# paninski-lab/eks

Hardware: AMD Instinct MI355X
Metric: frames*keypoints smoothed/s + achieved HBM GB/s fraction, singlecam 100k x 256 (higher is better)
Workload: dtype f32

## Files before the change

### eks_amd/csrc/eks_diag.hip

```cpp
#include <hip/hip_runtime.h>

#include <cstdlib>

#include "eks_diag_lane.hpp"
#include "eks_internal.hpp"

namespace eks {

struct LaneMap {
  int N, T, nc;
  int nt_log2;
  int ntile;
  int reverse;
};

__device__ __forceinline__ bool lane_coords(const LaneMap& L, int& n, int& j) {
  const int wave = blockIdx.x * (blockDim.x >> 6) + (threadIdx.x >> 6);
  const int lane = threadIdx.x & 63;
  const int tile = wave % L.ntile;
  const int cg = wave / L.ntile;
  const int nt = 1 << L.nt_log2;
  n = tile * nt + (lane & (nt - 1));
  j = cg * (64 >> L.nt_log2) + (lane >> L.nt_log2);
  return n < L.N && j < L.nc;
// ... 125 lines not shown
  }
  float eta = 0.f, J = 0.f;
  const int npass = (S.nblk + 63) / 64;
  for (int pass = npass - 1; pass >= 0; --pass) {
    const int q0 = pass * 64;
    const Elem<float> own = agg(q0 + lane);
    Elem<float> r = own;
#pragma unroll
    for (int off = 1; off < 64; off <<= 1) {
      const Elem<float> dn = shfl_down_elem(r, off);
      if (lane + off < 64) r = elem_combine(r, dn);
    }
    Elem<float> after = shfl_down_elem(r, 1);
    if (lane == 63) after = elem_identity<float>();
    float eq = eta, Jq = J;
    elem_back(after, eq, Jq);
    if (q0 + lane < S.nblk) {
      const size_t o = (size_t)(q0 + lane) * N + n;
      S.bEta[o] = eq;
      S.bJ[o] = Jq;
    }
    const Elem<float> all{__shfl(r.A, 0), __shfl(r.b, 0), __shfl(r.C, 0), __shfl(r.eta, 0), __shfl(r.J, 0)};
    elem_back(all, eta, J);
  }
}

__global__ __launch_bounds__(kScanCH* kScanCB) void diag_scan_local_kernel(int N, int nc, DiagWs W,
                                                                          ScanWs S) {
  __shared__ ScanLds L;
  const int cl = threadIdx.x % kScanCH, i = threadIdx.x / kScanCH;
  const int n = blockIdx.x * kScanCH + cl, j = blockIdx.y * kScanCB + i;
  const bool live = n < N && j < nc;
  L.put(i, cl, live ? load_elem(W, (size_t)j * N + n) : elem_identity<float>());
  __syncthreads();
  const int w = threadIdx.x >> 6, lane = threadIdx.x & 63;
  const Elem<float> own = L.get(lane, w);
  Elem<float> f = own, r = own;
#pragma unroll
  for (int off = 1; off < kScanCB; off <<= 1) {
    const Elem<float> up = shfl_up_elem(f, off), dn = shfl_down_elem(r, off);
    if (lane >= off) f = elem_combine(up, f);
    if (lane + off < kScanCB) r = elem_combine(r, dn);
  }
  Elem<float> excl = shfl_up_elem(f, 1), after = shfl_down_elem(r, 1);
  if (lane == 0) excl = elem_identity<float>();
  if (lane == kScanCB - 1) after = elem_identity<float>();
  const int nw = blockIdx.x * kScanCH + w;
  float m = 0.f, P = 0.f, eta = 0.f, J = 0.f;
  if (nw < N) {
    const size_t ob = (size_t)blockIdx.y * N + nw;
    m = S.bm[ob];
    P = S.bP[ob];
    eta = S.bEta[ob];
    J = S.bJ[ob];
  }
  elem_apply(excl, m, P);
  elem_back(after, eta, J);
  __syncthreads();
  L.A[lane][w] = m;
  L.b[lane][w] = P;
  L.C[lane][w] = eta;
  L.eta[lane][w] = J;
  __syncthreads();
  if (!live) return;
  const size_t o = (size_t)j * N + n;
  W.pm[o] = L.A[i][cl];
  W.pP[o] = L.b[i][cl];
  W.sEta[o] = L.C[i][cl];
  W.sJ[o] = L.eta[i][cl];
}

constexpr int kFW = 4;
static_assert(kFW == 4, "the fused kernels' LDS exchange, the group scan's slot sizes and the measured "
                        "thresholds in diag_smooth() assume four chunks per block");

struct BlockMap {
  int N, T, nc;
  int ntile;
  int ngrp;
  int reverse;
  int tile0;
};

struct BufferRows {
  __amdgpu_buffer_rsrc_t ry, rv;
  unsigned voff, row_bytes;
  __device__ __forceinline__ float load_y(int i) const {
    return __builtin_bit_cast(float, __builtin_amdgcn_raw_buffer_load_b32(ry, voff, (unsigned)i * row_bytes, 0));
  }
  __device__ __forceinline__ float load_var(int i) const {
    return __builtin_bit_cast(float, __builtin_amdgcn_raw_buffer_load_b32(rv, voff, (unsigned)i * row_bytes, 0));
  }
};

__device__ __forceinline__ __amdgpu_buffer_rsrc_t rows_rsrc(const float* base) {
  return __builtin_amdgcn_make_buffer_rsrc(const_cast<float*>(base), 0, 0x7FFFFFFF, 0x00020000);
}

constexpr int kAuxNt = 2;

template <int VS_ROW>
struct BufferStore {
  __amdgpu_buffer_rsrc_t rm, rV;
  unsigned voff, row_bytes;
  int d;
  __device__ __forceinline__ void operator()(int i, float m, float P) const {
    constexpr unsigned W = VS_ROW == 0 ? 1 : VS_ROW;
    const unsigned so = (unsigned)i * row_bytes;
    __builtin_amdgcn_raw_buffer_store_b32(__builtin_bit_cast(unsigned, m), rm, voff, so, kAuxNt);
    if constexpr (VS_ROW <= 1) {
      __builtin_amdgcn_raw_buffer_store_b32(__builtin_bit_cast(unsigned, P), rV, voff, so, kAuxNt);
    } else if constexpr (VS_ROW == 2) {
      typedef unsigned u2 __attribute__((ext_vector_type(2)));
      const u2 v = {__builtin_bit_cast(unsigned, d == 0 ? P : 0.0f), __builtin_bit_cast(unsigned, d == 1 ? P : 0.0f)};
      __builtin_amdgcn_raw_buffer_store_b64(v, rV, voff * 2, so * 2, kAuxNt);
    } else {
#pragma unroll
      for (unsigned e = 0; e < W; ++e)
        __builtin_amdgcn_raw_buffer_store_b32(__builtin_bit_cast(unsigned, (int)e == d ? P : 0.0f), rV,
                                              voff * W + 4 * e, so * W, kAuxNt);
    }
  }
};

template <int B, bool UNIT, bool RC>
__global__ __launch_bounds__(64 * kFW) void diag_summarize_blk_kernel(BlockMap L, DiagModel M, DiagWs W,
                                                                     ScanWs S,
                                                                     const float* __restrict__ y,
                                                                     const float* __restrict__ var) {
  __shared__ float sh[5][kFW][64];
  __shared__ int arrived;
  const int w = __builtin_amdgcn_readfirstlane(threadIdx.x >> 6), lane = threadIdx.x & 63;
  if (threadIdx.x == 0) arrived = 0;
  __syncthreads();
  const int tile = L.tile0 + blockIdx.x % L.ntile;
  int grp = blockIdx.x / L.ntile;
  if (L.reverse) grp = L.ngrp - 1 - grp;
  const int n = tile * 64 + lane, j = grp * kFW + w;
  Elem<float> e = elem_identity<float>();
  if (n < L.N && j < L.nc) {
    const ChainParams<float> p = load_chain_params(M, n);
    const int t0 = j * B, len = min(B, L.T - t0);
    const size_t first = (size_t)t0 * L.N + (size_t)tile * 64;
    const BufferRows rows{rows_rsrc(y + first), rows_rsrc(var + first), (unsigned)lane * 4, (unsigned)L.N * 4};
    float yy[B], rr[B];
    if (len == B) {
      load_rows<B, true>(rows, B, yy, rr);
      e = summarize_loaded<B, UNIT, true>(yy, rr, B, p);
    } else {
      load_rows<B, false>(rows, len, yy, rr);
      e = summarize_loaded<B, UNIT, false>(yy, rr, len, p);
    }
    if constexpr (!RC) {
      const size_t o = (size_t)j * L.N + n;
      W.eA[o] = e.A;
      W.eb[o] = e.b;
      W.eC[o] = e.C;
      W.eEta[o] = e.eta;
      W.eJ[o] = e.J;
    }
  }
  sh[0][w][lane] = e.A;
  sh[1][w][lane] = e.b;
  sh[2][w][lane] = e.C;
  sh[3][w][lane] = e.eta;
  sh[4][w][lane] = e.J;
  __builtin_amdgcn_fence(__ATOMIC_RELEASE, "workgroup");
  int ticket = 0;
  if (lane == 0) ticket = atomicAdd(&arrived, 1);
  ticket = __builtin_amdgcn_readfirstlane(ticket);
  if (ticket != kFW - 1 || n >= L.N) return;
  __builtin_amdgcn_fence(__ATOMIC_ACQUIRE, "workgroup");
  Elem<float> a{sh[0][0][lane], sh[1][0][lane], sh[2][0][lane], sh[3][0][lane], sh[4][0][lane]};
#pragma unroll
  for (int q = 1; q < kFW; ++q)
    a = elem_combine(a, Elem<float>{sh[0][q][lane], sh[1][q][lane], sh[2][q][lane], sh[3][q][lane],
                                    sh[4][q][lane]});
  const size_t o = (size_t)grp * L.N + n;
  S.gA[o] = a.A;
  S.gb[o] = a.b;
  S.gC[o] = a.C;
  S.gEta[o] = a.eta;
  S.gJ[o] = a.J;
}

template <int B, bool UNIT, int VS_ROW, bool RC>
__global__ __launch_bounds__(64 * kFW) void diag_replay_blk_kernel(BlockMap L, DiagModel M, DiagWs W,
                                                                  ScanWs S,
                                                                  const float* __restrict__ y,
                                                                  const float* __restrict__ var,
                                                                  float* __restrict__ ms,
                                                                  float* __restrict__ Vs) {
  const int w = __builtin_amdgcn_readfirstlane(threadIdx.x >> 6), lane = threadIdx.x & 63;
  const int tile = L.tile0 + blockIdx.x % L.ntile;
  int grp = blockIdx.x / L.ntile;
  if (L.reverse) grp = L.ngrp - 1 - grp;
  const int n = tile * 64 + lane, j = grp * kFW + w;
  const int j0 = grp * kFW, j1 = min(j0 + kFW, L.nc);
  constexpr int VW = VS_ROW == 0 ? 1 : VS_ROW;
  if constexpr (!RC) {
    if (n >= L.N || j >= L.nc) return;
    const ChainParams<float> p = load_chain_params(M, n);
    const int t0 = j * B;
    const int len = min(B, L.T - t0);
    const bool full = len == B;
    const size_t first = (size_t)t0 * L.N + (size_t)tile * 64;
    const BufferRows rows{rows_rsrc(y + first), rows_rsrc(var + first), (unsigned)lane * 4, (unsigned)L.N * 4};
    float v0[B], v1[B];
    if (full) load_rows<B, true>(rows, B, v0, v1);
    else load_rows<B, false>(rows, len, v0, v1);
    Elem<float> ef[kFW - 1];
#pragma unroll
    for (int q = 0; q < kFW - 1; ++q)
      if (j0 + q < j) ef[q] = load_elem(W, (size_t)(j0 + q) * L.N + n);
    const size_t ob = (size_t)grp * L.N + n;
    float m = S.bm[ob], P = S.bP[ob], eta = S.bEta[ob], J = S.bJ[ob];
#pragma unroll
    for (int q = 0; q < kFW - 1; ++q)
      if (j0 + q < j) elem_apply(ef[q], m, P);
    Elem<float> eb[kFW - 1];
#pragma unroll
    for (int q = 0; q < kFW - 1; ++q)
      if (j + 1 + q < j1) eb[q] = load_elem(W, (size_t)(j + 1 + q) * L.N + n);
    if (full) filter_loaded<B, UNIT, true>(v0, v1, B, p, m, P);
    else filter_loaded<B, UNIT, false>(v0, v1, len, p, m, P);
#pragma unroll
    for (int q = kFW - 2; q >= 0; --q)
      if (j + 1 + q < j1) elem_back(eb[q], eta, J);
    fuse_info(m, P, eta, J);
    const BufferStore<VS_ROW> st{rows_rsrc(ms + first), rows_rsrc(Vs + first * VW), (unsigned)lane * 4,
                                 (unsigned)L.N * 4, n % M.D};
    if (full) smooth_rows<B, UNIT, true>(v0, v1, B, p, m, P, st);
    else smooth_rows<B, UNIT, false>(v0, v1, len, p, m, P, st);
  } else {
    __shared__ float sh[5][kFW][64];
    const bool live = n < L.N && j < L.nc;
    ChainParams<float> p{1.f, 1.f, 0.f};
    const int t0 = j < L.nc ? j * B : 0;
    const int len = j < L.nc ? min(B, L.T - t0) : 0;
    const bool full = len == B;
    const size_t first = (size_t)t0 * L.N + (size_t)tile * 64;
    const BufferRows rows{rows_rsrc(y + first), rows_rsrc(var + first), (unsigned)lane * 4, (unsigned)L.N * 4};
    float v0[B], v1[B];
    Elem<float> own = elem_identity<float>();
    if (live) {
      p = load_chain_params(M, n);
      if (full) {
        load_rows<B, true>(rows, B, v0, v1);
        own = summarize_loaded<B, UNIT, true>(v0, v1, B, p);
      } else {
        load_rows<B, false>(rows, len, v0, v1);
        own = summarize_loaded<B, UNIT, false>(v0, v1, len, p);
      }
    }
    sh[0][w][lane] = own.A; sh[1][w][lane] = own.b; sh[2][w][lane] = own.C; sh[3][w][lane] = own.eta;
    sh[4][w][lane] = own.J;
    __syncthreads();
    if (!live) return;
    auto lds_elem = [&](int q) {
      return Elem<float>{sh[0][q][lane], sh[1][q][lane], sh[2][q][lane], sh[3][q][lane], sh[4][q][lane]};
    };
    const size_t ob = (size_t)grp * L.N + n;
    float m = S.bm[ob], P = S.bP[ob], eta = S.bEta[ob], J = S.bJ[ob];
#pragma unroll
    for (int q = 0; q < kFW - 1; ++q)
      if (q < w) elem_apply(lds_elem(q), m, P);
    Elem<float> eb[kFW - 1];
#pragma unroll
    for (int q = 0; q < kFW - 1; ++q)
      if (j + 1 + q < j1) eb[q] = lds_elem(w + 1 + q);
    if (full) filter_loaded<B, UNIT, true>(v0, v1, B, p, m, P);
    else filter_loaded<B, UNIT, false>(v0, v1, len, p, m, P);
#pragma unroll
    for (int q = kFW - 2; q >= 0; --q)
      if (j + 1 + q < j1) elem_back(eb[q], eta, J);
    fuse_info(m, P, eta, J);
    const BufferStore<VS_ROW> st{rows_rsrc(ms + first), rows_rsrc(Vs + first * VW), (unsigned)lane * 4,
                                 (unsigned)L.N * 4, n % M.D};
    if (full) smooth_rows<B, UNIT, true>(v0, v1, B, p, m, P, st);
    else smooth_rows<B, UNIT, false>(v0, v1, len, p, m, P, st);
  }
}

template <int PER, int CH>
__global__ __launch_bounds__(64 * CH) void diag_scan_groups_kernel(int N, int n0, int n1, DiagModel M, ScanWs S) {
  constexpr int NW = CH;
  __shared__ float tot[2][5][NW][CH];
  const int c = threadIdx.x % CH, slot = threadIdx.x / CH, w = threadIdx.x >> 6, lane = threadIdx.x & 63;
  const int lb = xcd_contiguous_block(blockIdx.x, gridDim.x);
  const int n = n0 + lb * CH + c;
  const int per = (S.nblk + 63) / 64;
  const int q0 = min(slot * per, S.nblk), q1 = min(q0 + per, S.nblk);
  const bool live = n < n1;
  auto agg = [&](int q) {
    const size_t o = (size_t)q * N + n;
    return Elem<float>{S.gA[o], S.gb[o], S.gC[o], S.gEta[o], S.gJ[o]};
  };
  Elem<float> own = elem_identity<float>();
  Elem<float> e[PER];
  if (live) {
    for (int b0 = q0; b0 < q1; b0 += PER) {
#pragma unroll
      for (int i = 0; i < PER; ++i)
        if (b0 + i < q1) e[i] = agg(b0 + i);
#pragma unroll
      for (int i = 0; i < PER; ++i)
        if (b0 + i < q1) own = elem_combine(own, e[i]);
    }
  }
  Elem<float> f = own, r = own;
#pragma unroll
  for (int off = CH; off < 64; off <<= 1) {
    const Elem<float> up = shfl_up_elem(f, off), dn = shfl_down_elem(r, off);
    if (lane >= off) f = elem_combine(up, f);
    if (lane + off < 64) r = elem_combine(r, dn);
  }
  if (lane >= 64 - CH) {
    tot[0][0][w][c] = f.A; tot[0][1][w][c] = f.b; tot[0][2][w][c] = f.C; tot[0][3][w][c] = f.eta; tot[0][4][w][c] = f.J;
  }
  if (lane < CH) {
    tot[1][0][w][c] = r.A; tot[1][1][w][c] = r.b; tot[1][2][w][c] = r.C; tot[1][3][w][c] = r.eta; tot[1][4][w][c] = r.J;
  }
  __syncthreads();
  if (!live) return;
  Elem<float> pre = elem_identity<float>(), post = elem_identity<float>();
  for (int v = 0; v < w; ++v)
    pre = elem_combine(pre, Elem<float>{tot[0][0][v][c], tot[0][1][v][c], tot[0][2][v][c], tot[0][3][v][c], tot[0][4][v][c]});
  for (int v = NW - 1; v > w; --v)
    post = elem_combine(Elem<float>{tot[1][0][v][c], tot[1][1][v][c], tot[1][2][v][c], tot[1][3][v][c], tot[1][4][v][c]}, post);
  Elem<float> fe = shfl_up_elem(f, CH), re = shfl_down_elem(r, CH);
  if (lane < CH) fe = elem_identity<float>();
  if (lane >= 64 - CH) re = elem_identity<float>();
  pre = elem_combine(pre, fe);
  post = elem_combine(re, post);
  float m, P;
  load_chain_prior(M, n, m, P);
  elem_apply(pre, m, P);
  float eta = 0.f, J = 0.f;
  elem_back(post, eta, J);
  const bool held = q1 - q0 <= PER;
  for (int b0 = q0; b0 < q1; b0 += PER) {
    if (!held) {
#pragma unroll
      for (int i = 0; i < PER; ++i)
        if (b0 + i < q1) e[i] = agg(b0 + i);
    }
#pragma unroll
    for (int i = 0; i < PER; ++i)
      if (b0 + i < q1) {
        const size_t o = (size_t)(b0 + i) * N + n;
        S.bm[o] = m;
        S.bP[o] = P;
        elem_apply(e[i], m, P);
      }
  }
  for (int b1 = q1; b1 > q0; b1 -= PER) {
    const int lo = max(q0, b1 - PER);
    if (!held) {
#pragma unroll
      for (int i = 0; i < PER; ++i)
        if (lo + i < b1) e[i] = agg(lo + i);
    }
#pragma unroll
    for (int i = PER - 1; i >= 0; --i)
      if (lo + i < b1) {
        const size_t o = (size_t)(lo + i) * N + n;
        S.bEta[o] = eta;
        S.bJ[o] = J;
        elem_back(e[i], eta, J);
      }
  }
}

#ifndef EKS_DIAG_CHUNK
#define EKS_DIAG_CHUNK 32
#endif
constexpr int kChunk = EKS_DIAG_CHUNK;

static inline size_t plane_bytes(int nc, int N) { return align_up((size_t)nc * N * sizeof(float), 256); }

size_t diag_smooth_workspace_bytes(int T, int N) {
  const int nc = (T + kChunk - 1) / kChunk;
  const int nblk = (nc + kFW - 1) / kFW;
  return 9 * plane_bytes(nc, N) + 9 * plane_bytes(nblk, N);
}

static LaneMap make_lane_map(int T, int N, int B) {
  LaneMap L;
  L.N = N;
  L.T = T;
  L.nc = (T + B - 1) / B;
  int nt_log2 = 0;
  while ((1 << nt_log2) < N && nt_log2 < 6) ++nt_log2;
  L.nt_log2 = nt_log2;
  L.ntile = (N + (1 << nt_log2) - 1) >> nt_log2;
  L.reverse = 0;
  return L;
}

template <bool UNIT>
static void launch_replay(int vs_row, dim3 grid, hipStream_t st, const LaneMap& L, const DiagModel& M,
                          const DiagWs& W, const float* y, const float* var, float* ms, float* Vs) {
#define EKS_REPLAY(R)                                                                             \
  case R:                                                                                         \
    hipLaunchKernelGGL((diag_replay_kernel<kChunk, UNIT, R>), grid, dim3(256), 0, st, L, M, W, y, \
                       var, ms, Vs);                                                              \
    break;
  switch (vs_row) {
    EKS_REPLAY(0)
    EKS_REPLAY(1)
    EKS_REPLAY(2)
    EKS_REPLAY(3)
    EKS_REPLAY(4)
    EKS_REPLAY(5)
    EKS_REPLAY(6)
    EKS_REPLAY(7)
    EKS_REPLAY(8)
  }
#undef EKS_REPLAY
}

int diag_smooth(const eks_dims_t& d, const float* y, const float* var, const DiagModel& M,
                float* ms, float* Vs, void* ws, size_t ws_bytes, hipStream_t st) {
  const int T = d.n_frames, D = d.state_dim, N = d.n_keypoints * D;
  const bool vs_diag = d.flags & EKS_FLAG_VS_DIAG;
  if (!vs_diag && D > 8) return EKS_ERR_UNSUPPORTED;
  if (ws_bytes < diag_smooth_workspace_bytes(T, N)) return EKS_ERR_WORKSPACE;
  const LaneMap Lf = make_lane_map(T, N, kChunk);
  const LaneMap& L = Lf;
  const size_t pb = plane_bytes(L.nc, N);
  char* base = static_cast<char*>(ws);
  DiagWs W;
  float** planes[9] = {&W.eA, &W.eb, &W.eC, &W.eEta, &W.eJ, &W.pm, &W.pP, &W.sEta, &W.sJ};
  for (int i = 0; i < 9; ++i) *planes[i] = reinterpret_cast<float*>(base + i * pb);
  const int ngrp_f = (L.nc + kFW - 1) / kFW;
  const bool in_range = (size_t)kChunk * N * (vs_diag ? 1 : D) * sizeof(float) < ((size_t)1 << 31);
  const bool fused = L.nt_log2 == 6 && in_range &&
                     (knob_set(KNOB_SMOOTH_UNFUSED) ? knob_int(KNOB_SMOOTH_UNFUSED, 0) == 0 : ngrp_f <= 1024);
  ScanWs S;
  S.nblk = fused ? (L.nc + kFW - 1) / kFW : (L.nc + kScanCB - 1) / kScanCB;
  const size_t sb = plane_bytes(S.nblk, N);
  float** splanes[9] = {&S.gA, &S.gb, &S.gC, &S.gEta, &S.gJ, &S.bm, &S.bP, &S.bEta, &S.bJ};
  for (int i = 0; i < 9; ++i) *splanes[i] = reinterpret_cast<float*>(base + 9 * pb + i * sb);
  const int vs_row = vs_diag ? 0 : D;
  const bool unit = d.flags & EKS_FLAG_UNIT_AC;
  const int k1_reverse = knob_int(KNOB_SUMMARIZE_REVERSE, 0) == 1 ? 1 : 0;
  const int k3_reverse = knob_set(KNOB_REPLAY_FORWARD) ? (knob_int(KNOB_REPLAY_FORWARD, 0) == 1 ? 0 : 1) : !k1_reverse;
  if (fused) {
    const bool rc_all = knob_set(KNOB_REPLAY_RECOMPUTE) ? knob_int(KNOB_REPLAY_RECOMPUTE, 0) == 1
                                                        : 5 * pb >= ((size_t)16 << 20);
    const int tp = L.ntile;
    for (int tile0 = 0; tile0 < L.ntile; tile0 += tp) {
    const int ntl = min(tp, L.ntile - tile0);
    const int n0 = tile0 * 64, Np = min(N - n0, ntl * 64);
    BlockMap Bm{N, T, L.nc, ntl, S.nblk, k1_reverse, tile0};
    const dim3 bgrid((unsigned)((long)Bm.ntile * Bm.ngrp)), bblock(64 * kFW);
    const bool rc = rc_all;
#define EKS_K1_BLK(UN)                                                                                  \
  do {                                                                                                  \
    if (rc)                                                                                             \
      hipLaunchKernelGGL((diag_summarize_blk_kernel<kChunk, UN, true>), bgrid, bblock, 0, st, Bm, M, W, \
                         S, y, var);                                                                    \
    else                                                                                                \
      hipLaunchKernelGGL((diag_summarize_blk_kernel<kChunk, UN, false>), bgrid, bblock, 0, st, Bm, M,   \
                         W, S, y, var);                                                                 \
  } while (0)
#define EKS_K3_BLK(UN, R)                                                                               \
  do {                                                                                                  \
    if (rc)                                                                                             \
      hipLaunchKernelGGL((diag_replay_blk_kernel<kChunk, UN, R, true>), bgrid, bblock, 0, st, Bm, M, W, \
                         S, y, var, ms, Vs);                                                            \
    else                                                                                                \
      hipLaunchKernelGGL((diag_replay_blk_kernel<kChunk, UN, R, false>), bgrid, bblock, 0, st, Bm, M,   \
                         W, S, y, var, ms, Vs);                                                         \
  } while (0)
    {
      ProfScope ps("diag_summarize", st);
      if (unit)
        EKS_K1_BLK(true);
      else
        EKS_K1_BLK(false);
    }
    {
      ProfScope ps("diag_scan", st);
      const bool ch4 = knob_set(KNOB_SCAN_CH) ? knob_int(KNOB_SCAN_CH, 4) == 4 : Np < 2048;
      const bool per8 = (S.nblk + 63) / 64 <= 8;
      const int Ne = n0 + Np;
      if (ch4) {
        if (per8)
          hipLaunchKernelGGL((diag_scan_groups_kernel<8, 4>), dim3((Np + 3) / 4), dim3(256), 0, st, N, n0, Ne, M, S);
        else
          hipLaunchKernelGGL((diag_scan_groups_kernel<16, 4>), dim3((Np + 3) / 4), dim3(256), 0, st, N, n0, Ne, M, S);
      } else {
        if (per8)
          hipLaunchKernelGGL((diag_scan_groups_kernel<8, 16>), dim3((Np + 15) / 16), dim3(1024), 0, st, N, n0, Ne, M, S);
        else
          hipLaunchKernelGGL((diag_scan_groups_kernel<16, 16>), dim3((Np + 15) / 16), dim3(1024), 0, st, N, n0, Ne, M, S);
      }
    }
    ProfScope ps("diag_replay", st);
    Bm.reverse = k3_reverse;
#define EKS_REPLAY_BLK(R)                                                                              \
  case R:                                                                                              \
    if (unit)                                                                                          \
      EKS_K3_BLK(true, R);                                                                             \
    else                                                                                               \
      EKS_K3_BLK(false, R);                                                                            \
    break;
    switch (vs_row) {
      EKS_REPLAY_BLK(0)
      EKS_REPLAY_BLK(1)
      EKS_REPLAY_BLK(2)
      EKS_REPLAY_BLK(3)
      EKS_REPLAY_BLK(4)
      EKS_REPLAY_BLK(5)
      EKS_REPLAY_BLK(6)
      EKS_REPLAY_BLK(7)
      EKS_REPLAY_BLK(8)
    }
    }
#undef EKS_REPLAY_BLK
#undef EKS_K3_BLK
#undef EKS_K1_BLK
    return hip_status(hipGetLastError());
  }

  const int cpw = 64 >> L.nt_log2;
  const long waves = (long)L.ntile * ((L.nc + cpw - 1) / cpw);
  const dim3 grid((unsigned)((waves + 3) / 4));
  {
    ProfScope ps("diag_summarize", st);
    LaneMap L = Lf;
    L.reverse = k1_reverse;
    if (unit)
      hipLaunchKernelGGL((diag_summarize_kernel<kChunk, true>), grid, dim3(256), 0, st, L, M, W, y, var);
    else
      hipLaunchKernelGGL((diag_summarize_kernel<kChunk, false>), grid, dim3(256), 0, st, L, M, W, y, var);
  }
  {
    ProfScope ps("diag_scan", st);
    const dim3 sgrid((N + kScanCH - 1) / kScanCH, S.nblk), sblock(kScanCH * kScanCB);
    hipLaunchKernelGGL(diag_scan_reduce_kernel, sgrid, sblock, 0, st, N, L.nc, W, S);
    hipLaunchKernelGGL(diag_scan_blocks_kernel, dim3((N + 3) / 4), dim3(256), 0, st, N, M, S);
    hipLaunchKernelGGL(diag_scan_local_kernel, sgrid, sblock, 0, st, N, L.nc, W, S);
  }
  {
    ProfScope ps("diag_replay", st);
    LaneMap L = Lf;
    L.reverse = k3_reverse;
    if (unit)
      launch_replay<true>(vs_row, grid, st, L, M, W, y, var, ms, Vs);
    else
      launch_replay<false>(vs_row, grid, st, L, M, W, y, var, ms, Vs);
  }
  return hip_status(hipGetLastError());
}

}

EKS_DEFINE_TOUCH(diag)
```

### eks_amd/csrc/eks_internal.hpp

```cpp
#pragma once
#include <hip/hip_runtime.h>

#include <cstddef>
#include <cstdint>

#include "../../include/eks_hip.h"

namespace eks {

struct DiagModel;

static inline size_t align_up(size_t x, size_t a) { return (x + a - 1) / a * a; }
static inline int hip_status(hipError_t e) { return e == hipSuccess ? EKS_OK : EKS_ERR_HIP_BASE - (int)e; }

__device__ __forceinline__ int xcd_contiguous_block(int b, int nb) {
  const int x = b & 7, i = b >> 3, q = nb >> 3, r = nb & 7;
  return x * q + (x < r ? x : r) + i;
}

enum Knob {
  KNOB_SMOOTH_UNFUSED, KNOB_SUMMARIZE_REVERSE, KNOB_REPLAY_FORWARD, KNOB_REPLAY_RECOMPUTE, KNOB_SCAN_CH,
  KNOB_DENSE_CHUNK, KNOB_NLL_NCL, KNOB_NLL_CHUNK, KNOB_NLL_CHUNK0, KNOB_NLL_WPB,
  KNOB_DENSE_LEGACY, KNOB_NLL_GRAD_UNFUSED, KNOB_NLL_GRAD_CHUNK,
  KNOB_DENSE_TREE_SCAN, KNOB_DENSE_DUAL_GRAD, KNOB_NLL_LEGACY, KNOB_MED_ROWS, KNOB_DW_CHUNK, KNOB_ADAM_PER_ITERATION, KNOB_MED_FINISH_THREADS, KNOB_MED_BRACKET_THREADS, KNOB_NLL_NOLAG, KNOB_NLL_GRAD_TREE, KNOB_ADAM_STREAM, KNOB_ADAM_LAG_RHO_PPM, KNOB_ADAM_LAG_HEAD, KNOB_COUNT
};
bool knob_set(Knob k);
int knob_int(Knob k, int dflt);

#define EKS_DEFINE_TOUCH(unit)                                                                              \
  namespace eks {                                                                                           \
  __global__ void touch_##unit##_kernel() {}                                                                \
  void touch_##unit() {                                                                                     \
    hipFuncAttributes a;                                                                                    \
    (void)hipFuncGetAttributes(&a, reinterpret_cast<const void*>(touch_##unit##_kernel));                   \
  }                                                                                                         \
  }
void touch_misc();
void touch_diag();
void touch_diag_nll();
void touch_dense();
void touch_dense_wave();
void touch_dense_wide();
void touch_loss();
void touch_loss_ar1();
void touch_multicam();
void touch_lag_adam();

class ProfScope {
 public:
  ProfScope(const char* name, hipStream_t st);
  ~ProfScope();

 private:
  const char* name_;
  hipStream_t st_;
  bool live_;
  hipEvent_t a_, b_;
};

size_t diag_smooth_workspace_bytes(int T, int N);
int diag_smooth(const eks_dims_t& d, const float* y, const float* var, const DiagModel& M,
                float* ms, float* Vs, void* ws, size_t ws_bytes, hipStream_t st);
size_t diag_nll_workspace_bytes(int T, int N, int n_cand);
struct AdamFuse;
int diag_nll(const eks_dims_t& d, const float* y, const double* rconst, const DiagModel& M,
             const double* s_cand, int n_cand, int per_keypoint, double* nll, double* dnll,
             void* ws, size_t ws_bytes, hipStream_t st, const AdamFuse* fuse = nullptr, double* s_out = nullptr,
             int32_t* idx_out = nullptr);
bool diag_nll_grad_tree(int T, int K, int D);
bool diag_nll_adam_persist_ok(int T, int K, int D, int n_blocks);
int diag_nll_adam_persist(const eks_dims_t& d, const float* y, const double* rconst, const DiagModel& M, int n_iters,
                          double* nll, double* dnll, const AdamFuse& F, int32_t* n_active, hipStream_t st);
bool diag_lag_adam_ok(int T, int K, int D, int n_blocks);
size_t diag_lag_adam_workspace_bytes(int T, int N);
int diag_lag_sums(const eks_dims_t& d, const float* y, const double* A, const AdamFuse* F, void* ws, size_t ws_bytes,
                  hipStream_t st);
int diag_lag_adam(const eks_dims_t& d, const float* y, const double* rconst, const DiagModel& M, int n_iters, double* nll,
                  double* dnll, const AdamFuse& F, void* ws, size_t ws_bytes, hipStream_t st);
size_t adam_extra_bytes(int N);
int32_t* nll_ws_tickets(void* ws, int T, int N, int n_cand);
int adam_prepare(int n_blocks, int K, const int32_t* offs, const int32_t* members, int32_t* kp_block,
                 int32_t* counter_a, int32_t* counter_b, hipStream_t st);

size_t diag_sample_workspace_bytes(int T, int N, int n_draws);
int diag_sample(const eks_dims_t& d, const float* y, const float* var, const DiagModel& M, int n_draws, uint64_t seed,
                int first_keypoint, int first_draw, const float* noise, float* ms, float* draws, void* ws,
                size_t ws_bytes, hipStream_t st);
int diag_sample_noise(int T, int N, int D, int n_draws, uint64_t seed, int first_keypoint, int first_draw, float* noise,
                      hipStream_t st);
struct DenseModel;
size_t dense_sample_workspace_bytes(int T, int K, int D, int O, int n_draws);
int dense_sample(const eks_dims_t& d, const float* y, const float* var, const DenseModel& M, int n_draws, uint64_t seed,
                 int first_keypoint, int first_draw, const float* noise, float* ms, float* draws, void* ws,
                 size_t ws_bytes, hipStream_t st);
int dense_sample_noise(int T, int K, int W, int n_draws, uint64_t seed, int first_keypoint, int first_draw, float* noise,
                       hipStream_t st);

struct DenseModel {
  const double *m0, *S0, *A, *C, *Q, *s;
};
bool diag_increments_covers(int T, int N);
size_t diag_increments_workspace_bytes(int T, int N);
int diag_increments(const eks_dims_t& d, const float* y, const float* var, const DiagModel& M, float* ms, float* Vs,
                    float* lag1, float* dmean, float* dV, void* ws, size_t ws_bytes, hipStream_t st);
size_t dense_increments_workspace_bytes(int T, int K, int D, int O);
int dense_increments(const eks_dims_t& d, const float* y, const float* var, const DenseModel& M, float* ms, float* Vs,
                     float* lag1, float* dmean, float* dV, void* ws, size_t ws_bytes, hipStream_t st);
// ... 116 lines not shown
```

### eks_amd/csrc/eks_profile.hip

```cpp
#include <hip/hip_runtime.h>

#include <cstdlib>
#include <cstring>
#include <mutex>
#include <vector>

#include "eks_internal.hpp"

namespace eks {

namespace {
struct KnobTable {
  bool set[KNOB_COUNT];
  int val[KNOB_COUNT];
  KnobTable() { load(); }
  int load() {
    static const char* const names[KNOB_COUNT] = {
        "EKS_SMOOTH_UNFUSED", "EKS_SUMMARIZE_REVERSE", "EKS_REPLAY_FORWARD", "EKS_REPLAY_RECOMPUTE", "EKS_SCAN_CH",
        "EKS_DENSE_CHUNK", "EKS_NLL_NCL", "EKS_NLL_CHUNK", "EKS_NLL_CHUNK0", "EKS_NLL_WPB",
        "EKS_DENSE_LEGACY", "EKS_NLL_GRAD_UNFUSED",
        "EKS_NLL_GRAD_CHUNK", "EKS_DENSE_TREE_SCAN", "EKS_DENSE_DUAL_GRAD", "EKS_NLL_LEGACY", "EKS_MED_ROWS", "EKS_DW_CHUNK", "EKS_ADAM_PER_ITERATION", "EKS_MED_FINISH_THREADS", "EKS_MED_BRACKET_THREADS", "EKS_NLL_NOLAG", "EKS_NLL_GRAD_TREE", "EKS_ADAM_STREAM", "EKS_ADAM_LAG_RHO_PPM", "EKS_ADAM_LAG_HEAD"};
    int n = 0;
    for (int i = 0; i < KNOB_COUNT; ++i) {
      const char* v = getenv(names[i]);
      set[i] = v != nullptr;
      val[i] = v ? atoi(v) : 0;
      n += set[i];
    }
    return n;
  }
};
KnobTable& knob_table() {
  static KnobTable t;
  return t;
}
}

bool knob_set(Knob k) { return knob_table().set[k]; }
int knob_int(Knob k, int dflt) { return knob_table().set[k] ? knob_table().val[k] : dflt; }

struct ProfEntry {
  const char* name;
  hipEvent_t a, b;
};
static int g_prof_level = 0;
static std::vector<ProfEntry> g_prof;
static std::vector<hipEvent_t> g_pool;
static std::mutex g_prof_mu;

static hipEvent_t take_event() {
  std::lock_guard<std::mutex> lk(g_prof_mu);
  if (!g_pool.empty()) {
    hipEvent_t e = g_pool.back();
    g_pool.pop_back();
    return e;
  }
  hipEvent_t e;
  hipEventCreate(&e);
  return e;
}

static bool scope_live(const char* name) {
  if (g_prof_level == 1) return true;
  if (g_prof_level != 2) return false;
  const size_t n = strlen(name);
  return (n >= 7 && strcmp(name + n - 7, "_replay") == 0) || strcmp(name, "diag_nll_summarize") == 0;
}

ProfScope::ProfScope(const char* name, hipStream_t st) : name_(name), st_(st), live_(scope_live(name)) {
  if (!live_) return;
  a_ = take_event();
  b_ = take_event();
  hipEventRecord(a_, st_);
}
ProfScope::~ProfScope() {
  if (!live_) return;
  hipEventRecord(b_, st_);
  std::lock_guard<std::mutex> lk(g_prof_mu);
  g_prof.push_back({name_, a_, b_});
}

}

extern "C" {

int eks_knobs_reload(void) { return eks::knob_table().load(); }

int eks_profile_enable(int on) {
  eks::g_prof_level = on < 0 ? 0 : on > 2 ? 1 : on;
  return EKS_OK;
}

int eks_profile_drain(char* names, size_t names_bytes, float* ms, int32_t max_n) {
  std::lock_guard<std::mutex> lk(eks::g_prof_mu);
  int n = 0;
  size_t off = 0;
  for (auto& e : eks::g_prof) {
    hipEventSynchronize(e.b);
    float t = 0.f;
    hipEventElapsedTime(&t, e.a, e.b);
    eks::g_pool.push_back(e.a);
    eks::g_pool.push_back(e.b);
    const size_t len = strlen(e.name) + 1;
    if (n < max_n && names && ms && off + len <= names_bytes) {
// ... 11 lines not shown
```

Measured before the change: 50.65 billion.

## Add windowed replay that smooths chunks from local halos instead of full scan

Adds a windowed smoothing path for long sequences (T at least 32768, on by default). Each block filters and smooths a group of chunks using only a small halo of neighbouring chunk summaries, and relies on the filter forgetting its initial state. This avoids the summarize and group-scan passes and their extra HBM traffic. A probe kernel classifies chains whose forgetting is too slow, and the windowed kernel flags windows where the halo did not contract below tolerance. Those chains and windows are then recomputed exactly through gated summarize, scan and masked replay kernels, which adds a probe launch and some complexity in exchange.

```diff
diff --git a/eks_amd/csrc/eks_diag.hip b/eks_amd/csrc/eks_diag.hip
--- a/eks_amd/csrc/eks_diag.hip
+++ b/eks_amd/csrc/eks_diag.hip
@@ -231,6 +231,28 @@
   int tile0;
 };
 
+#ifndef EKS_WIN_G
+#define EKS_WIN_G 8
+#endif
+constexpr int kWinG = EKS_WIN_G;
+constexpr int kWinH = 2;
+constexpr int kWinW = kWinG + 2 * kWinH;
+constexpr float kWinTol = 0x1p-30f;
+constexpr int kWinDefault = 1;
+constexpr int kWinMinT = 32768;
+constexpr int kProbeWin = 8;
+constexpr int kProbeLen = 64;
+static_assert(kWinG % kFW == 0, "the four chunks of an exact-replay block belong to one window group");
+static_assert(kWinG >= kWinH, "only the first window group's halo is cut by frame 0");
+
+struct WinWs {
+  unsigned char* slow;
+  unsigned char* fail;
+  int* gate;
+  int nwg;
+  int nan_bad;
+};
+
 struct BufferRows {
   __amdgpu_buffer_rsrc_t ry, rv;
   unsigned voff, row_bytes;
@@ -276,9 +298,11 @@
 __global__ __launch_bounds__(64 * kFW) void diag_summarize_blk_kernel(BlockMap L, DiagModel M, DiagWs W,
                                                                      ScanWs S,
                                                                      const float* __restrict__ y,
-                                                                     const float* __restrict__ var) {
+                                                                     const float* __restrict__ var,
+                                                                     const int* __restrict__ gate) {
   __shared__ float sh[5][kFW][64];
   __shared__ int arrived;
+  if (gate && gate[L.tile0 + blockIdx.x % L.ntile] == 0) return;
   const int w = __builtin_amdgcn_readfirstlane(threadIdx.x >> 6), lane = threadIdx.x & 63;
   if (threadIdx.x == 0) arrived = 0;
   __syncthreads();
@@ -333,13 +357,11 @@
   S.gJ[o] = a.J;
 }
 
-template <int B, bool UNIT, int VS_ROW, bool RC>
-__global__ __launch_bounds__(64 * kFW) void diag_replay_blk_kernel(BlockMap L, DiagModel M, DiagWs W,
-                                                                  ScanWs S,
-                                                                  const float* __restrict__ y,
-                                                                  const float* __restrict__ var,
-                                                                  float* __restrict__ ms,
-                                                                  float* __restrict__ Vs) {
+template <int B, bool UNIT, int VS_ROW, bool MASKED>
+__device__ __forceinline__ void replay_recompute_block(const BlockMap& L, const DiagModel& M, const ScanWs& S,
+                                                       const WinWs& Wn, const float* __restrict__ y,
+                                                       const float* __restrict__ var, float* __restrict__ ms,
+                                                       float* __restrict__ Vs) {
   const int w = __builtin_amdgcn_readfirstlane(threadIdx.x >> 6), lane = threadIdx.x & 63;
   const int tile = L.tile0 + blockIdx.x % L.ntile;
   int grp = blockIdx.x / L.ntile;
@@ -347,7 +369,163 @@
   const int n = tile * 64 + lane, j = grp * kFW + w;
   const int j0 = grp * kFW, j1 = min(j0 + kFW, L.nc);
   constexpr int VW = VS_ROW == 0 ? 1 : VS_ROW;
-  if constexpr (!RC) {
+  __shared__ float sh[5][kFW][64];
+  bool keep = true;
+  if constexpr (MASKED) {
+    if (Wn.gate[tile] == 0) return;
+    keep = n < L.N && (Wn.slow[n] | Wn.fail[(size_t)(j0 / kWinG) * L.N + n]) != 0;
+    if (__ballot(keep) == 0) return;
+  }
+  const bool live = n < L.N && j < L.nc;
+  ChainParams<float> p{1.f, 1.f, 0.f};
+  const int t0 = j < L.nc ? j * B : 0;
+  const int len = j < L.nc ? min(B, L.T - t0) : 0;
+  const bool full = len == B;
+  const size_t first = (size_t)t0 * L.N + (size_t)tile * 64;
+  const BufferRows rows{rows_rsrc(y + first), rows_rsrc(var + first), (unsigned)lane * 4, (unsigned)L.N * 4};
+  float v0[B], v1[B];
+  Elem<float> own = elem_identity<float>();
+  if (live) {
+    p = load_chain_params(M, n);
+    if (full) {
+      load_rows<B, true>(rows, B, v0, v1);
+      own = summarize_loaded<B, UNIT, true>(v0, v1, B, p);
+    } else {
+      load_rows<B, false>(rows, len, v0, v1);
+      own = summarize_loaded<B, UNIT, false>(v0, v1, len, p);
+    }
+  }
+  sh[0][w][lane] = own.A; sh[1][w][lane] = own.b; sh[2][w][lane] = own.C; sh[3][w][lane] = own.eta;
+  sh[4][w][lane] = own.J;
+  __syncthreads();
+  if (!live) return;
+  auto lds_elem = [&](int q) {
+    return Elem<float>{sh[0][q][lane], sh[1][q][lane], sh[2][q][lane], sh[3][q][lane], sh[4][q][lane]};
+  };
+  const size_t ob = (size_t)grp * L.N + n;
+  float m = S.bm[ob], P = S.bP[ob], eta = S.bEta[ob], J = S.bJ[ob];
+#pragma unroll
+  for (int q = 0; q < kFW - 1; ++q)
+    if (q < w) elem_apply(lds_elem(q), m, P);
+  Elem<float> eb[kFW - 1];
+#pragma unroll
+  for (int q = 0; q < kFW - 1; ++q)
+    if (j + 1 + q < j1) eb[q] = lds_elem(w + 1 + q);
+  if (full) filter_loaded<B, UNIT, true>(v0, v1, B, p, m, P);
+  else filter_loaded<B, UNIT, false>(v0, v1, len, p, m, P);
+#pragma unroll
+  for (int q = kFW - 2; q >= 0; --q)
+    if (j + 1 + q < j1) elem_back(eb[q], eta, J);
+  fuse_info(m, P, eta, J);
+  const BufferStore<VS_ROW> st{rows_rsrc(ms + first), rows_rsrc(Vs + first * VW), (unsigned)lane * 4,
+                               (unsigned)L.N * 4, n % M.D};
+  if (!MASKED || keep) {
+    if (full) smooth_rows<B, UNIT, true>(v0, v1, B, p, m, P, st);
+    else smooth_rows<B, UNIT, false>(v0, v1, len, p, m, P, st);
+  }
+}
+
+template <int B, bool UNIT, int VS_ROW>
+__device__ __forceinline__ void replay_window_block(const BlockMap& L, const DiagModel& M, const WinWs& Wn,
+                                                    const float* __restrict__ y, const float* __restrict__ var,
+                                                    float* __restrict__ ms, float* __restrict__ Vs) {
+  __shared__ float sh[5][kWinW][64];
+  __shared__ float shy[64];
+  const int w = __builtin_amdgcn_readfirstlane(threadIdx.x >> 6), lane = threadIdx.x & 63;
+  const int tile = L.tile0 + blockIdx.x % L.ntile;
+  int wg = blockIdx.x / L.ntile;
+  if (L.reverse) wg = Wn.nwg - 1 - wg;
+  const int n = tile * 64 + lane;
+  constexpr int VW = VS_ROW == 0 ? 1 : VS_ROW;
+  const bool slow = n >= L.N || (Wn.slow != nullptr && Wn.slow[n] != 0);
+  if (__ballot(!slow) == 0) return;
+  const int jh0 = wg * kWinG - kWinH;
+  const int j = jh0 + w;
+  const bool valid = j >= 0 && j < L.nc;
+  const bool live = n < L.N && valid;
+  ChainParams<float> p{1.f, 1.f, 0.f};
+  const int t0 = valid ? j * B : 0;
+  const int len = valid ? min(B, L.T - t0) : 0;
+  const bool full = len == B;
+  const size_t first = (size_t)t0 * L.N + (size_t)tile * 64;
+  const BufferRows rows{rows_rsrc(y + first), rows_rsrc(var + first), (unsigned)lane * 4, (unsigned)L.N * 4};
+  float v0[B], v1[B];
+  Elem<float> own = elem_identity<float>();
+  float y0 = 0.f;
+  if (live) {
+    p = load_chain_params(M, n);
+    if (full) {
+      load_rows<B, true>(rows, B, v0, v1);
+      y0 = v0[0];
+      own = summarize_loaded<B, UNIT, true>(v0, v1, B, p);
+    } else {
+      load_rows<B, false>(rows, len, v0, v1);
+      y0 = v0[0];
+      own = summarize_loaded<B, UNIT, false>(v0, v1, len, p);
+    }
+  }
+  sh[0][w][lane] = own.A; sh[1][w][lane] = own.b; sh[2][w][lane] = own.C; sh[3][w][lane] = own.eta;
+  sh[4][w][lane] = own.J;
+  if (w == 0) shy[lane] = y0;
+  __syncthreads();
+  const int wo = w - kWinH;
+  if (wo < 0 || wo >= kWinG || !live) return;
+  auto lds_elem = [&](int q) {
+    return Elem<float>{sh[0][q][lane], sh[1][q][lane], sh[2][q][lane], sh[3][q][lane], sh[4][q][lane]};
+  };
+  const bool cut_front = jh0 <= 0, cut_back = (wg + 1) * kWinG + kWinH >= L.nc;
+  Elem<float> hf = lds_elem(0), hb = lds_elem(kWinH + kWinG);
+#pragma unroll
+  for (int q = 1; q < kWinH; ++q) {
+    hf = elem_combine(hf, lds_elem(q));
+    hb = elem_combine(hb, lds_elem(kWinH + kWinG + q));
+  }
+  float m, P;
+  load_chain_prior(M, n, m, P);
+  if (!cut_front) m = UNIT ? shy[lane] : shy[lane] * rcp(p.c);
+  const bool good = !slow && fabsf(m) <= 3e38f && (cut_front || fabsf(hf.A) <= kWinTol) &&
+                    (cut_back || fabsf(hb.A) <= kWinTol);
+  if (!good && !slow && wo == 0 && Wn.fail != nullptr) {
+    Wn.fail[(size_t)wg * L.N + n] = 1;
+    atomicOr(&Wn.gate[tile], 1);
+  }
+  elem_apply(hf, m, P);
+  for (int q = 0; q < wo; ++q) elem_apply(lds_elem(kWinH + q), m, P);
+  if (full) filter_loaded<B, UNIT, true>(v0, v1, B, p, m, P);
+  else filter_loaded<B, UNIT, false>(v0, v1, len, p, m, P);
+  float eta = 0.f, J = 0.f;
+  elem_back(hb, eta, J);
+  for (int q = kWinG - 1; q > wo; --q) elem_back(lds_elem(kWinH + q), eta, J);
+  fuse_info(m, P, eta, J);
+  if (Wn.nan_bad && !good) m = P = __builtin_nanf("");
+  const BufferStore<VS_ROW> st{rows_rsrc(ms + first), rows_rsrc(Vs + first * VW), (unsigned)lane * 4,
+                               (unsigned)L.N * 4, n % M.D};
+  if (good || Wn.nan_bad) {
+    if (full) smooth_rows<B, UNIT, true>(v0, v1, B, p, m, P, st);
+    else smooth_rows<B, UNIT, false>(v0, v1, len, p, m, P, st);
+  }
+}
+
+constexpr int kFormElems = 0;
+constexpr int kFormRecompute = 1;
+constexpr int kFormWindow = 2;
+
+template <int B, bool UNIT, int VS_ROW, int FORM>
+__global__ __launch_bounds__(FORM == kFormWindow ? 64 * kWinW : 64 * kFW) void diag_replay_blk_kernel(
+    BlockMap L, DiagModel M, DiagWs W, ScanWs S, WinWs Wn, const float* __restrict__ y, const float* __restrict__ var,
+    float* __restrict__ ms, float* __restrict__ Vs) {
+  if constexpr (FORM == kFormWindow) {
+    replay_window_block<B, UNIT, VS_ROW>(L, M, Wn, y, var, ms, Vs);
+  } else if constexpr (FORM == kFormRecompute) {
+    replay_recompute_block<B, UNIT, VS_ROW, false>(L, M, S, Wn, y, var, ms, Vs);
+  } else {
+    const int w = __builtin_amdgcn_readfirstlane(threadIdx.x >> 6), lane = threadIdx.x & 63;
+    const int tile = L.tile0 + blockIdx.x % L.ntile;
+    int grp = blockIdx.x / L.ntile;
+    if (L.reverse) grp = L.ngrp - 1 - grp;
+    const int n = tile * 64 + lane, j = grp * kFW + w;
+    const int j0 = grp * kFW, j1 = min(j0 + kFW, L.nc);
+    constexpr int VW = VS_ROW == 0 ? 1 : VS_ROW;
     if (n >= L.N || j >= L.nc) return;
     const ChainParams<float> p = load_chain_params(M, n);
     const int t0 = j * B;
@@ -381,60 +559,63 @@
                                  (unsigned)L.N * 4, n % M.D};
     if (full) smooth_rows<B, UNIT, true>(v0, v1, B, p, m, P, st);
     else smooth_rows<B, UNIT, false>(v0, v1, len, p, m, P, st);
-  } else {
-    __shared__ float sh[5][kFW][64];
-    const bool live = n < L.N && j < L.nc;
-    ChainParams<float> p{1.f, 1.f, 0.f};
-    const int t0 = j < L.nc ? j * B : 0;
-    const int len = j < L.nc ? min(B, L.T - t0) : 0;
-    const bool full = len == B;
-    const size_t first = (size_t)t0 * L.N + (size_t)tile * 64;
-    const BufferRows rows{rows_rsrc(y + first), rows_rsrc(var + first), (unsigned)lane * 4, (unsigned)L.N * 4};
-    float v0[B], v1[B];
-    Elem<float> own = elem_identity<float>();
-    if (live) {
-      p = load_chain_params(M, n);
-      if (full) {
-        load_rows<B, true>(rows, B, v0, v1);
-        own = summarize_loaded<B, UNIT, true>(v0, v1, B, p);
-      } else {
-        load_rows<B, false>(rows, len, v0, v1);
-        own = summarize_loaded<B, UNIT, false>(v0, v1, len, p);
-      }
-    }
-    sh[0][w][lane] = own.A; sh[1][w][lane] = own.b; sh[2][w][lane] = own.C; sh[3][w][lane] = own.eta;
-    sh[4][w][lane] = own.J;
-    __syncthreads();
-    if (!live) return;
-    auto lds_elem = [&](int q) {
-      return Elem<float>{sh[0][q][lane], sh[1][q][lane], sh[2][q][lane], sh[3][q][lane], sh[4][q][lane]};
-    };
-    const size_t ob = (size_t)grp * L.N + n;
-    float m = S.bm[ob], P = S.bP[ob], eta = S.bEta[ob], J = S.bJ[ob];
-#pragma unroll
-    for (int q = 0; q < kFW - 1; ++q)
-      if (q < w) elem_apply(lds_elem(q), m, P);
-    Elem<float> eb[kFW - 1];
-#pragma unroll
-    for (int q = 0; q < kFW - 1; ++q)
-      if (j + 1 + q < j1) eb[q] = lds_elem(w + 1 + q);
-    if (full) filter_loaded<B, UNIT, true>(v0, v1, B, p, m, P);
-    else filter_loaded<B, UNIT, false>(v0, v1, len, p, m, P);
-#pragma unroll
-    for (int q = kFW - 2; q >= 0; --q)
-      if (j + 1 + q < j1) elem_back(eb[q], eta, J);
-    fuse_info(m, P, eta, J);
-    const BufferStore<VS_ROW> st{rows_rsrc(ms + first), rows_rsrc(Vs + first * VW), (unsigned)lane * 4,
-                                 (unsigned)L.N * 4, n % M.D};
-    if (full) smooth_rows<B, UNIT, true>(v0, v1, B, p, m, P, st);
-    else smooth_rows<B, UNIT, false>(v0, v1, len, p, m, P, st);
-  }
+  }
+}
+
+template <int B, bool UNIT, int VS_ROW>
+__global__ __launch_bounds__(64 * kFW) void diag_replay_exact_kernel(BlockMap L, DiagModel M, ScanWs S, WinWs Wn,
+                                                                    const float* __restrict__ y,
+                                                                    const float* __restrict__ var,
+                                                                    float* __restrict__ ms,
+                                                                    float* __restrict__ Vs) {
+  replay_recompute_block<B, UNIT, VS_ROW, true>(L, M, S, Wn, y, var, ms, Vs);
+}
+
+__global__ __launch_bounds__(64 * kProbeWin) void diag_window_probe_kernel(int N, int T, DiagModel M, WinWs Wn,
+                                                                          const float* __restrict__ var,
+                                                                          int classify) {
+  __shared__ int bad[kProbeWin][64];
+  const int w = __builtin_amdgcn_readfirstlane(threadIdx.x >> 6), lane = threadIdx.x & 63;
+  const int tile = blockIdx.x, n = tile * 64 + lane;
+  for (int i = threadIdx.x; i < Wn.nwg * 64; i += 64 * kProbeWin) {
+    const int c = tile * 64 + (i & 63);
+    if (c < N) Wn.fail[(size_t)(i >> 6) * N + c] = 0;
+  }
+  int s = 0;
+  if (classify && n < N) {
+    const ChainParams<float> p = load_chain_params(M, n);
+    const int t0 = (int)((long long)w * (T - kProbeLen) / (kProbeWin - 1));
+    const float* v = var + (size_t)t0 * N + n;
+    float r[kProbeLen];
+#pragma unroll
+    for (int i = 0; i < kProbeLen; ++i) r[i] = v[(size_t)i * N];
+    float A = 1.f, C = 0.f;
+#pragma unroll
+    for (int i = 0; i < kProbeLen; ++i) {
+      const float ri = clip_var(r[i]);
+      const float rg = ri * rcp(ri + C * p.c * p.c);
+      A = p.times_a(A * rg);
+      C = p.times_a2(C * rg) + p.q_s;
+    }
+    s = !(fabsf(A) <= kWinTol);
+  }
+  bad[w][lane] = s;
+  __syncthreads();
+  if (w != 0) return;
+#pragma unroll
+  for (int q = 1; q < kProbeWin; ++q) s |= bad[q][lane];
+  if (n < N) Wn.slow[n] = (unsigned char)s;
+  const bool any = __ballot(s != 0) != 0;
+  if (lane == 0) Wn.gate[tile] = any ? 1 : 0;
 }
 
 template <int PER, int CH>
-__global__ __launch_bounds__(64 * CH) void diag_scan_groups_kernel(int N, int n0, int n1, DiagModel M, ScanWs S) {
+__global__ __launch_bounds__(64 * CH) void diag_scan_groups_kernel(int N, int n0, int n1, DiagModel M, ScanWs S,
+                                                                  const int* __restrict__ gate) {
   constexpr int NW = CH;
   __shared__ float tot[2][5][NW][CH];
+  static_assert(64 % CH == 0, "a block's chains lie in one 64-chain tile (n0 is a multiple of 64)");
+  if (gate && gate[(n0 + xcd_contiguous_block(blockIdx.x, gridDim.x) * CH) >> 6] == 0) return;
   const int c = threadIdx.x % CH, slot = threadIdx.x / CH, w = threadIdx.x >> 6, lane = threadIdx.x & 63;
   const int lb = xcd_contiguous_block(blockIdx.x, gridDim.x);
   const int n = n0 + lb * CH + c;
@@ -528,10 +709,16 @@
 
 static inline size_t plane_bytes(int nc, int N) { return align_up((size_t)nc * N * sizeof(float), 256); }
 
+static inline size_t win_slow_bytes(int N) { return align_up((size_t)N, 256); }
+static inline size_t win_fail_bytes(int nc, int N) { return align_up((size_t)((nc + kWinG - 1) / kWinG) * N, 256); }
+static inline size_t win_bytes(int nc, int N) {
+  return win_slow_bytes(N) + win_fail_bytes(nc, N) + align_up((size_t)((N + 63) / 64) * sizeof(int), 256);
+}
+
 size_t diag_smooth_workspace_bytes(int T, int N) {
   const int nc = (T + kChunk - 1) / kChunk;
   const int nblk = (nc + kFW - 1) / kFW;
-  return 9 * plane_bytes(nc, N) + 9 * plane_bytes(nblk, N);
+  return 9 * plane_bytes(nc, N) + 9 * plane_bytes(nblk, N) + win_bytes(nc, N);
 }
 
 static LaneMap make_lane_map(int T, int N, int B) {
@@ -595,6 +782,21 @@
   const bool unit = d.flags & EKS_FLAG_UNIT_AC;
   const int k1_reverse = knob_int(KNOB_SUMMARIZE_REVERSE, 0) == 1 ? 1 : 0;
   const int k3_reverse = knob_set(KNOB_REPLAY_FORWARD) ? (knob_int(KNOB_REPLAY_FORWARD, 0) == 1 ? 0 : 1) : !k1_reverse;
+  const int win_mode = knob_int(KNOB_SMOOTH_WINDOW, kWinDefault);
+  const int win_min_t = max(kProbeLen, knob_int(KNOB_SMOOTH_WINDOW_MIN_T, kWinMinT));
+  const bool windowed = fused && win_mode != 0 && T >= win_min_t;
+  WinWs Wn{nullptr, nullptr, nullptr, (L.nc + kWinG - 1) / kWinG, 0};
+  if (windowed) {
+    char* wb = base + 9 * pb + 9 * sb;
+    if (win_mode == 2) {
+      Wn.nan_bad = 1;
+    } else {
+      Wn.slow = reinterpret_cast<unsigned char*>(wb);
+      Wn.fail = reinterpret_cast<unsigned char*>(wb + win_slow_bytes(N));
+      Wn.gate = reinterpret_cast<int*>(wb + win_slow_bytes(N) + win_fail_bytes(L.nc, N));
+    }
+  }
+  const int* gate = windowed ? Wn.gate : nullptr;
   if (fused) {
     const bool rc_all = knob_set(KNOB_REPLAY_RECOMPUTE) ? knob_int(KNOB_REPLAY_RECOMPUTE, 0) == 1
                                                         : 5 * pb >= ((size_t)16 << 20);
@@ -604,25 +806,63 @@
     const int n0 = tile0 * 64, Np = min(N - n0, ntl * 64);
     BlockMap Bm{N, T, L.nc, ntl, S.nblk, k1_reverse, tile0};
     const dim3 bgrid((unsigned)((long)Bm.ntile * Bm.ngrp)), bblock(64 * kFW);
-    const bool rc = rc_all;
+    const bool rc = rc_all || windowed;
 #define EKS_K1_BLK(UN)                                                                                  \
   do {                                                                                                  \
     if (rc)                                                                                             \
       hipLaunchKernelGGL((diag_summarize_blk_kernel<kChunk, UN, true>), bgrid, bblock, 0, st, Bm, M, W, \
-                         S, y, var);                                                                    \
+                         S, y, var, gate);                                                              \
     else                                                                                                \
       hipLaunchKernelGGL((diag_summarize_blk_kernel<kChunk, UN, false>), bgrid, bblock, 0, st, Bm, M,   \
-                         W, S, y, var);                                                                 \
+                         W, S, y, var, gate);                                                           \
   } while (0)
 #define EKS_K3_BLK(UN, R)                                                                               \
   do {                                                                                                  \
-    if (rc)                                                                                             \
-      hipLaunchKernelGGL((diag_replay_blk_kernel<kChunk, UN, R, true>), bgrid, bblock, 0, st, Bm, M, W, \
-                         S, y, var, ms, Vs);                                                            \
+    if (windowed)                                                                                       \
+      hipLaunchKernelGGL((diag_replay_exact_kernel<kChunk, UN, R>), bgrid, bblock, 0, st, Bm, M, S, Wn, \
+                         y, var, ms, Vs);                                                               \
+    else if (rc)                                                                                        \
+      hipLaunchKernelGGL((diag_replay_blk_kernel<kChunk, UN, R, kFormRecompute>), bgrid, bblock, 0, st, \
+                         Bm, M, W, S, Wn, y, var, ms, Vs);                                              \
     else                                                                                                \
-      hipLaunchKernelGGL((diag_replay_blk_kernel<kChunk, UN, R, false>), bgrid, bblock, 0, st, Bm, M,   \
-                         W, S, y, var, ms, Vs);                                                         \
+      hipLaunchKernelGGL((diag_replay_blk_kernel<kChunk, UN, R, kFormElems>), bgrid, bblock, 0, st, Bm, \
+                         M, W, S, Wn, y, var, ms, Vs);                                                  \
   } while (0)
+#define EKS_K3_WIN(UN, R)                                                                               \
+  hipLaunchKernelGGL((diag_replay_blk_kernel<kChunk, UN, R, kFormWindow>), wgrid, dim3(64 * kWinW), 0,  \
+                     st, Bw, M, W, S, Wn, y, var, ms, Vs)
+#define EKS_REPLAY_WIN(R)                                                                              \
+  case R:                                                                                              \
+    if (unit)                                                                                          \
+      EKS_K3_WIN(true, R);                                                                             \
+    else                                                                                               \
+      EKS_K3_WIN(false, R);                                                                            \
+    break;
+    if (windowed) {
+      if (win_mode != 2) {
+        ProfScope ps("diag_window_probe", st);
+        hipLaunchKernelGGL(diag_window_probe_kernel, dim3(ntl), dim3(64 * kProbeWin), 0, st, N, T, M, Wn, var,
+                           knob_int(KNOB_SMOOTH_WINDOW_PROBE, 1) != 0 ? 1 : 0);
+      }
+      {
+        ProfScope ps("diag_replay", st);
+        BlockMap Bw = Bm;
+        Bw.reverse = k3_reverse;
+        const dim3 wgrid((unsigned)((long)Bw.ntile * Wn.nwg));
+        switch (vs_row) {
+          EKS_REPLAY_WIN(0)
+          EKS_REPLAY_WIN(1)
+          EKS_REPLAY_WIN(2)
+          EKS_REPLAY_WIN(3)
+          EKS_REPLAY_WIN(4)
+          EKS_REPLAY_WIN(5)
+          EKS_REPLAY_WIN(6)
+          EKS_REPLAY_WIN(7)
+          EKS_REPLAY_WIN(8)
+        }
+      }
+      if (win_mode == 2) continue;
+    }
     {
       ProfScope ps("diag_summarize", st);
       if (unit)
@@ -637,17 +877,17 @@
       const int Ne = n0 + Np;
       if (ch4) {
         if (per8)
-          hipLaunchKernelGGL((diag_scan_groups_kernel<8, 4>), dim3((Np + 3) / 4), dim3(256), 0, st, N, n0, Ne, M, S);
+          hipLaunchKernelGGL((diag_scan_groups_kernel<8, 4>), dim3((Np + 3) / 4), dim3(256), 0, st, N, n0, Ne, M, S, gate);
         else
-          hipLaunchKernelGGL((diag_scan_groups_kernel<16, 4>), dim3((Np + 3) / 4), dim3(256), 0, st, N, n0, Ne, M, S);
+          hipLaunchKernelGGL((diag_scan_groups_kernel<16, 4>), dim3((Np + 3) / 4), dim3(256), 0, st, N, n0, Ne, M, S, gate);
       } else {
         if (per8)
-          hipLaunchKernelGGL((diag_scan_groups_kernel<8, 16>), dim3((Np + 15) / 16), dim3(1024), 0, st, N, n0, Ne, M, S);
+          hipLaunchKernelGGL((diag_scan_groups_kernel<8, 16>), dim3((Np + 15) / 16), dim3(1024), 0, st, N, n0, Ne, M, S, gate);
         else
-          hipLaunchKernelGGL((diag_scan_groups_kernel<16, 16>), dim3((Np + 15) / 16), dim3(1024), 0, st, N, n0, Ne, M, S);
+          hipLaunchKernelGGL((diag_scan_groups_kernel<16, 16>), dim3((Np + 15) / 16), dim3(1024), 0, st, N, n0, Ne, M, S, gate);
       }
     }
-    ProfScope ps("diag_replay", st);
+    ProfScope ps(windowed ? "diag_replay_exact" : "diag_replay", st);
     Bm.reverse = k3_reverse;
 #define EKS_REPLAY_BLK(R)                                                                              \
   case R:                                                                                              \
@@ -669,6 +909,8 @@
     }
     }
 #undef EKS_REPLAY_BLK
+#undef EKS_REPLAY_WIN
+#undef EKS_K3_WIN
 #undef EKS_K3_BLK
 #undef EKS_K1_BLK
     return hip_status(hipGetLastError());
diff --git a/eks_amd/csrc/eks_internal.hpp b/eks_amd/csrc/eks_internal.hpp
--- a/eks_amd/csrc/eks_internal.hpp
+++ b/eks_amd/csrc/eks_internal.hpp
@@ -22,7 +22,8 @@
   KNOB_SMOOTH_UNFUSED, KNOB_SUMMARIZE_REVERSE, KNOB_REPLAY_FORWARD, KNOB_REPLAY_RECOMPUTE, KNOB_SCAN_CH,
   KNOB_DENSE_CHUNK, KNOB_NLL_NCL, KNOB_NLL_CHUNK, KNOB_NLL_CHUNK0, KNOB_NLL_WPB,
   KNOB_DENSE_LEGACY, KNOB_NLL_GRAD_UNFUSED, KNOB_NLL_GRAD_CHUNK,
-  KNOB_DENSE_TREE_SCAN, KNOB_DENSE_DUAL_GRAD, KNOB_NLL_LEGACY, KNOB_MED_ROWS, KNOB_DW_CHUNK, KNOB_ADAM_PER_ITERATION, KNOB_MED_FINISH_THREADS, KNOB_MED_BRACKET_THREADS, KNOB_NLL_NOLAG, KNOB_NLL_GRAD_TREE, KNOB_ADAM_STREAM, KNOB_ADAM_LAG_RHO_PPM, KNOB_ADAM_LAG_HEAD, KNOB_COUNT
+  KNOB_DENSE_TREE_SCAN, KNOB_DENSE_DUAL_GRAD, KNOB_NLL_LEGACY, KNOB_MED_ROWS, KNOB_DW_CHUNK, KNOB_ADAM_PER_ITERATION, KNOB_MED_FINISH_THREADS, KNOB_MED_BRACKET_THREADS, KNOB_NLL_NOLAG, KNOB_NLL_GRAD_TREE, KNOB_ADAM_STREAM, KNOB_ADAM_LAG_RHO_PPM, KNOB_ADAM_LAG_HEAD,
+  KNOB_SMOOTH_WINDOW, KNOB_SMOOTH_WINDOW_MIN_T, KNOB_SMOOTH_WINDOW_PROBE, KNOB_COUNT
 };
 bool knob_set(Knob k);
 int knob_int(Knob k, int dflt);
diff --git a/eks_amd/csrc/eks_profile.hip b/eks_amd/csrc/eks_profile.hip
--- a/eks_amd/csrc/eks_profile.hip
+++ b/eks_amd/csrc/eks_profile.hip
@@ -19,7 +19,8 @@
         "EKS_SMOOTH_UNFUSED", "EKS_SUMMARIZE_REVERSE", "EKS_REPLAY_FORWARD", "EKS_REPLAY_RECOMPUTE", "EKS_SCAN_CH",
         "EKS_DENSE_CHUNK", "EKS_NLL_NCL", "EKS_NLL_CHUNK", "EKS_NLL_CHUNK0", "EKS_NLL_WPB",
         "EKS_DENSE_LEGACY", "EKS_NLL_GRAD_UNFUSED",
-        "EKS_NLL_GRAD_CHUNK", "EKS_DENSE_TREE_SCAN", "EKS_DENSE_DUAL_GRAD", "EKS_NLL_LEGACY", "EKS_MED_ROWS", "EKS_DW_CHUNK", "EKS_ADAM_PER_ITERATION", "EKS_MED_FINISH_THREADS", "EKS_MED_BRACKET_THREADS", "EKS_NLL_NOLAG", "EKS_NLL_GRAD_TREE", "EKS_ADAM_STREAM", "EKS_ADAM_LAG_RHO_PPM", "EKS_ADAM_LAG_HEAD"};
+        "EKS_NLL_GRAD_CHUNK", "EKS_DENSE_TREE_SCAN", "EKS_DENSE_DUAL_GRAD", "EKS_NLL_LEGACY", "EKS_MED_ROWS", "EKS_DW_CHUNK", "EKS_ADAM_PER_ITERATION", "EKS_MED_FINISH_THREADS", "EKS_MED_BRACKET_THREADS", "EKS_NLL_NOLAG", "EKS_NLL_GRAD_TREE", "EKS_ADAM_STREAM", "EKS_ADAM_LAG_RHO_PPM", "EKS_ADAM_LAG_HEAD",
+        "EKS_SMOOTH_WINDOW", "EKS_SMOOTH_WINDOW_MIN_T", "EKS_SMOOTH_WINDOW_PROBE"};
     int n = 0;
     for (int i = 0; i < KNOB_COUNT; ++i) {
       const char* v = getenv(names[i]);
```

New measurement: 55.09 billion (median of 6 runs). 8.8% higher.
